# LouChao98/VLGAE

Measured on AMD Instinct MI355X. Metric: sentences/sec, batched inside-outside L=40 B=256, higher is better.
Workload: dtype f32

## Files before the change

vlgae_amd/csrc/vlg_dp_core.h:

```cpp
#pragma once

#if defined(__HIPCC__)
#include <hip/hip_runtime.h>
#define VLG_HD __device__ __forceinline__
#define VLG_HOSTDEV __host__ __device__ inline
#define VLG_HDM __device__ __forceinline__
#define VLG_HOSTDEV_M __host__ __device__
#define VLG_EXP(x) __builtin_amdgcn_exp2f(x)
#define VLG_LOG(x) __builtin_amdgcn_logf(x)
#define VLG_BITS2F(u) __uint_as_float(u)
#define VLG_ATOMIC_ADD(p, v) atomicAdd((p), (v))
#else
#include <cmath>
#include <cstddef>
#include <cstdint>
#include <cstring>
#define VLG_HD static inline
#define VLG_HOSTDEV static inline
#define VLG_HDM inline
#define VLG_HOSTDEV_M
#define VLG_EXP(x) exp2f(x)
#define VLG_LOG(x) log2f(x)
struct float2 { float x, y; };
static inline float2 make_float2(float a, float b) { float2 r; r.x = a; r.y = b; return r; }
static inline float vlg_bits2f(uint32_t u) { float f; std::memcpy(&f, &u, 4); return f; }
#define VLG_BITS2F(u) vlg_bits2f(u)
#define VLG_ATOMIC_ADD(p, v) (*(p) += (v))
#endif

#define VLG_NEGINF (-1e12f)
#define VLG_SR_LOG 0
#define VLG_SR_MAX 1
#define VLG_LOWEST (-3.0e38f)
#if defined(VLG_STAMP) && defined(__HIPCC__) && VLG_STAMP != 2
#define VLG_STAMP_AT(x, k) (x).stamp(k)
#else
#define VLG_STAMP_AT(x, k) ((void)0)
#endif
#if defined(VLG_STAMP) && defined(__HIPCC__)
#define VLG_WSTAMP(x, pass, w, k) (x).wstamp((pass), (w), (k))
#else
#define VLG_WSTAMP(x, pass, w, k) ((void)0)
#endif
#define VLG_LOG2E 1.44269504088896340736f
#define VLG_LN2 0.69314718055994530942f

namespace vlg {

struct F32In {
    using T = float;
    static VLG_HDM float ld(const T* p, size_t i) { return p[i]; }
    static VLG_HDM float2 ld2(const T* p, size_t i) { return make_float2(p[i], p[i + 1]); }
};
#define VLG_POT_FLOOR (-1e30f)
VLG_HD float pot_clamp(float x) { return x > VLG_POT_FLOOR ? x : VLG_POT_FLOOR; }
VLG_HD float2 pot_clamp2(float2 x) { return make_float2(pot_clamp(x.x), pot_clamp(x.y)); }
struct BF16In {
    using T = uint16_t;
    static VLG_HDM float ld(const T* p, size_t i) { return VLG_BITS2F((uint32_t)p[i] << 16); }
    static VLG_HDM float2 ld2(const T* p, size_t i) {
        return make_float2(VLG_BITS2F((uint32_t)p[i] << 16), VLG_BITS2F((uint32_t)p[i + 1] << 16));
    }
};

struct ValSumIn {
    using T = float2;
    static VLG_HDM float ld(const T* p, size_t i) { const float2 v = p[i]; return v.x + v.y; }
};

VLG_HOSTDEV int chart_pitch(int N) { return (N + 1) | 1; }

VLG_HD int dec_idx(int dir, int val, int z) { return (dir * 2 + val) * 2 + z; }

struct DmvCtx {
    int Ne;
    int len;
    int P;
    float2* C;
    float2* I;
    float2* C2;
    float2* I2;
    float* S;
    float* gCc;
    float2* gCi;
    float2* gI;
    float* decs;
    float* gdecs;
    unsigned char* bpS;
    unsigned char* bpC;
    bool walk;
};

template <int SR>
VLG_HD float adj_w(float g, float t, float out, int r, int bp) {
    if (SR == VLG_SR_MAX) return r == bp ? g : 0.f;
    return g * VLG_EXP(fminf(t - out, 0.f));
}

VLG_HD void upd_max(float& m, int& am, float t, int r) {
    if (t > m) { m = t; am = r; }
}

template <int SR>
VLG_HD float fold_term(float m, float s, int am, float t, int rt, bool t_first, int& bp) {
    if (SR == VLG_SR_MAX) {
        const bool take = t_first ? (t >= m) : (t > m);
        bp = take ? rt : am;
        return take ? t : m;
    }
    bp = 0;
    const float d = m - t, e = VLG_EXP(-fabsf(d));
    const float S = d >= 0.f ? s + e : fmaf(s, e, 1.f);
    return fmaxf(m, t) + VLG_LOG(S);
}

#ifndef VLG_DP_LANES_FW
#define VLG_DP_LANES_FW 256
#endif
#ifndef VLG_DP_LANES_BW
#define VLG_DP_LANES_BW 256
#endif
VLG_HD int group_log2(int spans, int w, int nt, int budget) {
    const int cap = budget < nt ? budget : nt;
    int lg = 0;
    while (lg < 6 && (1 << lg) < w && spans * (2 << lg) <= cap) ++lg;
    return lg;
}
#ifndef VLG_MIRROR_RIGHT
#define VLG_MIRROR_RIGHT 1
#endif
#define VLG_GROUP_LOG2_FW(spans, w, nt) group_log2(spans, w, nt, VLG_DP_LANES_FW)
#define VLG_GROUP_LOG2_BW(spans, w, nt) group_log2(spans, w, nt, 512)

struct Sched {
    int first[8];
};
VLG_HD Sched make_sched(int Ne, int lanes, int budget) {
    const int cap = budget < lanes ? budget : lanes;
    Sched s;
    s.first[0] = 1;
    for (int k = 1; k <= 6; ++k) {
        int a = (1 << (k - 1)) + 1, b = Ne - (cap >> k);
        int f = a > b ? a : b;
        if (f < s.first[k - 1]) f = s.first[k - 1];
        s.first[k] = f < Ne ? f : Ne;
    }
    s.first[7] = Ne;
    return s;
}

constexpr int kSpansGeneral = 0, kSpansLong = 1, kSpansShort = 2;
constexpr int kShortN = 41;
constexpr int group_log2_c(int spans, int w, int cap) {
    int lg = 0;
    while (lg < 6 && (1 << lg) < w && spans * (2 << lg) <= cap) ++lg;
    return lg;
}
constexpr bool short_sentence_ok(int n_max, int cap) {
    for (int ne = 2; ne <= n_max; ++ne)
        for (int w = 1; w < ne; ++w) {
            const int lg = group_log2_c(ne - w, w, cap);
            if (((w + (1 << lg) - 1) >> lg) > 3) return false;
        }
    return true;
}
constexpr int short_tmax(int lg_want, int n_max, int cap) {
    int m = 1;
    for (int ne = 2; ne <= n_max; ++ne)
        for (int w = 1; w < ne; ++w) {
            const int lg = group_log2_c(ne - w, w, cap), t = (w + (1 << lg) - 1) >> lg;
            if (lg == lg_want && t > m) m = t;
        }
    return m;
}
static_assert(short_sentence_ok(kShortN, VLG_DP_LANES_FW) && short_sentence_ok(kShortN, VLG_DP_LANES_BW),
// ... 338 lines not shown
                xb[u] = Cf[eB + 2 * rc];
                o_gi[u] = c.gI[eV + rc];
                o_c[u] = c.gCc[eU + rP];
                o_ga[u] = gCif[eA + 2 * rc];
                o_gb[u] = gCif[eB + 2 * rc];
            }
#pragma unroll
            for (int u = 0; u < TU; ++u) {
                const int r = r0 + u * G;
                const bool ok = r < w;
                w0[u] = ok ? adj_w<SR>(gc.x, uu[u] + vv[u].x, oc.x, r, b0) : 0.f;
                w1[u] = ok ? adj_w<SR>(gc.y, uu[u] + vv[u].y, oc.y, r, b1) : 0.f;
            }
            if (!CHUNKED) {
                self[0] = adj_w<SR>(gc.x, su + sv.x, oc.x, selfr, b0);
                self[1] = adj_w<SR>(gc.y, su + sv.y, oc.y, selfr, b1);
            }
            x.lockstep();
            if (!CHUNKED) {
                gi = make_float2(gi_old.x + self[0], gi_old.y + self[1]);
                gs = gi.x + gi.y;
            }
#pragma unroll
            for (int u = 0; u < TU; ++u) {
                const int r = r0 + u * G;
                if (live && r < w) {
                    const float ws = adj_w<SR>(gs, xa[u] + xb[u], Sv, r, bs);
                    if (r != selfr) c.gI[eV + r] = make_float2(o_gi[u].x + w0[u], o_gi[u].y + w1[u]);
                    c.gCc[eU + VLG_MUL24(r, P)] = o_c[u] + (w0[u] + w1[u]);
                    gCif[eA + 2 * r] = o_ga[u] + ws;
                    gCif[eB + 2 * r] = o_gb[u] + ws;
                }
            }
        }
        if (live && rr == 0) c.gI[kO] = gi;
        return;
    }
    for (int r = rr; r < w; r += G) {
        const int rP = VLG_MUL24(r, P);
        const float a = Cf[2 * (eU + rP) + 1];
        const float2 v = c.I[eV + r];
        const float q0 = adj_w<SR>(gc.x, a + v.x, oc.x, r, b0);
        const float q1 = adj_w<SR>(gc.y, a + v.y, oc.y, r, b1);
        if (r != selfr && live) { const float2 t = c.gI[eV + r]; c.gI[eV + r] = make_float2(t.x + q0, t.y + q1); }
        if (live) c.gCc[eU + rP] += q0 + q1;
    }
    self[0] = adj_w<SR>(gc.x, su + sv.x, oc.x, selfr, b0);
    self[1] = adj_w<SR>(gc.y, su + sv.y, oc.y, selfr, b1);
    x.lockstep();
    const float2 gi = make_float2(gi_old.x + self[0], gi_old.y + self[1]);
    const float gs = gi.x + gi.y;
    for (int r = rr; r < w; r += G) {
        const float ws = adj_w<SR>(gs, Cf[eA + 2 * r] + Cf[eB + 2 * r], Sv, r, bs);
        if (live) {
            gCif[eA + 2 * r] += ws;
            gCif[eB + 2 * r] += ws;
        }
    }
    if (live && rr == 0) c.gI[kO] = gi;
}

template <int TM>
struct BwVals {
    float2 oc, sv, vv[TM];
    float Sv, su, uu[TM], xa[TM], xb[TM];
};

template <typename T>
VLG_HD T addr_ld(const char* p, int off = 0) { return *reinterpret_cast<const T*>(p + off); }
template <typename T>
VLG_HD void addr_st(char* p, int off, T v) { *reinterpret_cast<T*>(p + off) = v; }

struct BwAddr {
    const char *vC, *vI, *vS, *vSU, *vUU, *vVV, *vXA, *vXB;
    char *aGc, *aGi, *aI, *aUU, *aVV, *aXA, *aXB;
    int sO8, sO4, sSU, sUU8, sUU4, sVV, sXB;
    int gp8, gp4;
    VLG_HDM void step_vals() { vC += sO8; vI += sO8; vS += sO4; vSU += sSU; vUU += sUU8; vVV += sVV; vXB += sXB; }
    VLG_HDM void step_adj() { aGc += sO4; aGi += sO8; aI += sO8; aUU += sUU4; aVV += sVV; aXB += sXB; }
};

template <int G, typename X>
VLG_HD BwAddr dmv_bw_addr(const DmvCtx& c, int w, int D, int rr, bool right, X& x) {
    const int P = c.P, DW = D + VLG_MUL24(w, P), q = D + rr, qP = D + VLG_MUL24(rr, P);
    const int kO = right ? D + w + 1 : DW, kS = right ? D + w : DW;
    const int iSU = right ? DW + w + 1 : D, iUU = right ? qP + P + w + 1 : qP, iVV = right ? q + 2 : DW + rr;
    const int iXA = q + 1, iXB = DW + rr + 1;
    const int cA = right ? 0 : 4, cB = right ? 4 : 0;
    const char *C = reinterpret_cast<const char*>(c.C), *I = reinterpret_cast<const char*>(c.I), *S = reinterpret_cast<const char*>(c.S);
    char *gCc = reinterpret_cast<char*>(c.gCc), *gCi = reinterpret_cast<char*>(c.gCi), *gI = reinterpret_cast<char*>(c.gI);
    BwAddr a;
    a.vC = x.pin(C + 8 * kO);
    a.vI = x.pin(I + 8 * kO);
    a.vS = x.pin(S + 4 * kS);
    a.vSU = x.pin(C + 8 * iSU + 4);
    a.vUU = x.pin(C + 8 * iUU + 4);
    a.vVV = x.pin(I + 8 * iVV);
    a.vXA = x.pin(C + 8 * iXA + cA);
    a.vXB = x.pin(C + 8 * iXB + cB);
    a.aGc = x.pin(gCc + 4 * kO);
    a.aGi = x.pin(gCi + 8 * kO);
    a.aI = x.pin(gI + 8 * kO);
    a.aUU = x.pin(gCc + 4 * iUU);
    a.aVV = x.pin(gI + 8 * iVV);
    a.aXA = x.pin(gCi + 8 * iXA + cA);
    a.aXB = x.pin(gCi + 8 * iXB + cB);
    a.sO8 = x.uniform(right ? -8 : -8 * P);
    a.sO4 = x.uniform(right ? -4 : -4 * P);
    a.sSU = x.uniform(right ? -8 * (P + 1) : 0);
    a.sUU8 = x.uniform(right ? -8 : 0);
    a.sUU4 = x.uniform(right ? -4 : 0);
    a.sVV = x.uniform(right ? 0 : -8 * P);
    a.sXB = -8 * P;
    a.gp8 = 8 * G * P;
    a.gp4 = 4 * G * P;
    return a;
}

template <int DIR>
struct FwAddr {
    const char *eA, *eB, *eU, *eV, *cX;
    char *oI, *oC, *oS;
    int p8, p4;
    int gp8;
    VLG_HDM void step() {
        eB += p8;
        if (DIR == 0) { eV += p8; oI += p8; oC += p8; oS += p4; }
        else { eU += 8; oI += 8; oC += 8; oS += 4; cX += p8 + 8; }
    }
};

template <int DIR, int G, bool TAPE, typename X>
VLG_HD FwAddr<DIR> dmv_fw_addr(const DmvCtx& c, int w, int D, int rr, X& x) {
    const int P = c.P, DW = D + VLG_MUL24(w, P), q = D + rr, qP = D + VLG_MUL24(rr, P);
    const int kO = DIR == 0 ? DW : D + w + 1;
    const char* C = reinterpret_cast<const char*>(c.C);
    const char* I = reinterpret_cast<const char*>(c.I);
    FwAddr<DIR> a;
    a.eA = x.pin(C + 8 * (q + 1) + (DIR == 0 ? 4 : 0));
    a.eB = x.pin(C + 8 * (DW + rr + 1) + (DIR == 0 ? 0 : 4));
    a.eU = x.pin(C + 8 * (DIR == 0 ? qP : qP + P + w + 1) + 4);
    a.eV = x.pin(I + 8 * (DIR == 0 ? DW + rr : q + 2));
    a.cX = x.pin(C + 8 * (DIR == 0 ? D : DW + w + 1) + 4);
    a.oI = x.pin(reinterpret_cast<char*>(c.I) + 8 * kO);
    a.oC = x.pin(reinterpret_cast<char*>(c.C) + 8 * kO);
    a.oS = nullptr;
    if constexpr (TAPE) a.oS = x.pin(reinterpret_cast<char*>(c.S) + 4 * (DIR == 0 ? DW : D + w));
    a.p8 = x.uniform(8 * P);
    a.p4 = x.uniform(4 * P);
    a.gp8 = 8 * G * P;
    return a;
}

template <int SR, bool BWD, int DIR, int G, int TU, typename X>
VLG_HD void dmv_fw_span_p(const DmvCtx& c, const FwAddr<DIR>& a, int w, bool live, bool root_row, int rr, int D, X& x) {
    const float2 aX = addr_ld<float2>(a.oI);
    const float cX = addr_ld<float>(a.cX);
    float m[3], s[3] = {0.f, 0.f, 0.f};
    int am[3];
    float t[TU][3];
#pragma unroll
    for (int u = 0; u < TU; ++u) {
        const int r = rr + u * G;
        const float av = addr_ld<float>(a.eA, u * G * 8), bv = addr_ld<float>(a.eB, u * G * 8);
        const float uu = addr_ld<float>(a.eU, u * a.gp8);
        const float2 vv = addr_ld<float2>(a.eV, u * G * 8);
        const bool last = u == TU - 1;
        const bool v0 = last ? r < w : true;
        const bool v1 = DIR == 0 ? (v0 && (u == 0 ? r >= 1 : true)) : (last ? r <= w - 2 : true);
        t[u][0] = v0 ? av + bv : VLG_LOWEST;
        t[u][1] = v1 ? uu + vv.x : VLG_LOWEST;
        t[u][2] = v1 ? uu + vv.y : VLG_LOWEST;
    }
#pragma unroll
    for (int k = 0; k < 3; ++k) {
        m[k] = t[0][k];
        am[k] = rr;
        if (SR == VLG_SR_LOG) {
#pragma unroll
            for (int u = 1; u < TU; ++u) m[k] = fmaxf(m[k], t[u][k]);
        } else {
#pragma unroll
            for (int u = 1; u < TU; ++u)
                if (t[u][k] > m[k]) { m[k] = t[u][k]; am[k] = rr + u * G; }
        }
    }
    if (SR == VLG_SR_MAX) x.template allreduce_argmax<3>(m, am, G);
    else x.template allreduce_max<3>(m, G);
    if (SR == VLG_SR_LOG) {
#pragma unroll
        for (int k = 0; k < 3; ++k) {
            s[k] = VLG_EXP(t[0][k] - m[k]);
#pragma unroll
            for (int u = 1; u < TU; ++u) s[k] += VLG_EXP(t[u][k] - m[k]);
        }
        x.template allreduce_sum<3>(s, G);
    }
    const float Sv = SR == VLG_SR_LOG ? m[0] + VLG_LOG(s[0]) : m[0];
    const float2 In = make_float2(aX.x + Sv, aX.y + Sv);
    int b0, b1;
    float Cx = fold_term<SR>(m[1], s[1], am[1], cX + In.x, DIR == 0 ? 0 : w - 1, DIR == 0, b0);
    float Cy = fold_term<SR>(m[2], s[2], am[2], cX + In.y, DIR == 0 ? 0 : w - 1, DIR == 0, b1);
    if (DIR == 1 && root_row && w != c.len) { Cx = VLG_NEGINF; Cy = VLG_NEGINF; }
    if (live && rr == 0) {
        addr_st(a.oI, 0, In);
        addr_st(a.oC, 0, make_float2(Cx, Cy));
        if (BWD) {
            if (SR != VLG_SR_MAX) addr_st(a.oS, 0, Sv);
            if (SR == VLG_SR_MAX) {
                const int DW = D + VLG_MUL24(w, c.P), kO = DIR == 0 ? DW : D + w + 1, kS = DIR == 0 ? DW : D + w;
                c.bpS[kS] = (unsigned char)am[0];
                c.bpC[kO * 2] = (unsigned char)b0;
                c.bpC[kO * 2 + 1] = (unsigned char)b1;
            }
        }
    }
}

template <int SR, bool BWD, int DIR, int LG, int TU, typename X>
VLG_HD void dmv_fw_piece_p(const DmvCtx& c, FwAddr<DIR>& a, int wa, int wb, int slot, int wslot, int rr, int D, X& x) {
    constexpr int G = 1 << LG;
    for (int w = wa; w < wb; ++w) {
        const int spans = x.uniform(c.Ne - w);
        const bool live = slot < spans;
        if (!(X::kSkipDeadWaves && wslot >= spans)) dmv_fw_span_p<SR, BWD, DIR, G, TU>(c, a, w, live, slot == 0, rr, D, x);
        a.step();
        VLG_WSTAMP(x, 0, w, 0);
        x.sync();
        VLG_WSTAMP(x, 0, w, 1);
    }
}

template <int SR, bool BWD, int DIR, int LG, int TM, typename X>
VLG_HD void dmv_fw_dir_p(const DmvCtx& c, int w0, int w1, int t, X& x) {
    constexpr int G = 1 << LG;
    const int rr = t & (G - 1), slot = t >> LG, wslot = (t & ~63) >> LG;
    const int D = slot < c.Ne - w0 ? VLG_MUL24(slot, c.P + 1) : 0;
    FwAddr<DIR> a = dmv_fw_addr<DIR, G, BWD && SR != VLG_SR_MAX>(c, w0, D, rr, x);
#pragma unroll
    for (int k = 1; k <= TM; ++k) {
        const int lo = (k - 1) * G + 1, hi = k == TM ? w1 : k * G + 1;
        const int wa = w0 > lo ? w0 : lo, wb = w1 < hi ? w1 : hi;
        if (k == 1) dmv_fw_piece_p<SR, BWD, DIR, LG, 1>(c, a, wa, wb, slot, wslot, rr, D, x);
        else if (k == 2) dmv_fw_piece_p<SR, BWD, DIR, LG, 2>(c, a, wa, wb, slot, wslot, rr, D, x);
        else dmv_fw_piece_p<SR, BWD, DIR, LG, 3>(c, a, wa, wb, slot, wslot, rr, D, x);
    }
}

template <int SR, bool BWD, int LG, int TM, typename X>
VLG_HD void dmv_fw_segment_p(const DmvCtx& c, int w0, int w1, int tid, int nt, X& x) {
    static_assert(TM >= 1 && TM <= 3, "dmv_fw_dir_p's pieces end at three split points per lane");
    if (w1 <= w0) return;
    const int nd = nt >> 1;
    const bool right = x.uniform(tid >= nd);
    const int t = dir_lane<VLG_MIRROR_RIGHT>(tid, nd, right);
    if (right) dmv_fw_dir_p<SR, BWD, 1, LG, TM>(c, w0, w1, t, x);
    else dmv_fw_dir_p<SR, BWD, 0, LG, TM>(c, w0, w1, t, x);
}

template <int G, int TM, bool XA = true>
VLG_HD void dmv_bw_load_vals(const BwAddr& a, BwVals<TM>& v) {
    v.oc = addr_ld<float2>(a.vC);
    v.Sv = addr_ld<float>(a.vS);
    v.su = addr_ld<float>(a.vSU);
    v.sv = addr_ld<float2>(a.vI);
#pragma unroll
    for (int u = 0; u < TM; ++u) {
        v.uu[u] = addr_ld<float>(a.vUU, u * a.gp8);
        v.vv[u] = addr_ld<float2>(a.vVV, u * G * 8);
        if constexpr (XA) v.xa[u] = addr_ld<float>(a.vXA, u * G * 8);
        v.xb[u] = addr_ld<float>(a.vXB, u * G * 8);
    }
}

template <int TM>
struct BwAdj {
    float ga, o_c[TM], o_gb[TM];
    float2 gb, gi_old, o_gi[TM];
    float e0[TM], e1[TM], es[TM], s0, s1;
};

template <int G, int TM, typename X>
VLG_HD void dmv_bw_span_p1(const BwAddr& a, X& x, const BwVals<TM>& v, BwAdj<TM>& s) {
    s.ga = addr_ld<float>(a.aGc);
    s.gb = addr_ld<float2>(a.aGi);
    s.gi_old = addr_ld<float2>(a.aI);
#pragma unroll
    for (int u = 0; u < TM; ++u) {
        s.o_gi[u] = addr_ld<float2>(a.aVV, u * G * 8);
        s.o_c[u] = addr_ld<float>(a.aUU, u * a.gp4);
        s.o_gb[u] = addr_ld<float>(a.aXB, u * G * 8);
    }
#pragma unroll
    for (int u = 0; u < TM; ++u) {
        s.e0[u] = VLG_EXP(fminf(v.uu[u] + v.vv[u].x - v.oc.x, 0.f));
        s.e1[u] = VLG_EXP(fminf(v.uu[u] + v.vv[u].y - v.oc.y, 0.f));
        s.es[u] = VLG_EXP(fminf(v.xa[u] + v.xb[u] - v.Sv, 0.f));
    }
    s.s0 = VLG_EXP(fminf(v.su + v.sv.x - v.oc.x, 0.f));
    s.s1 = VLG_EXP(fminf(v.su + v.sv.y - v.oc.y, 0.f));
#pragma unroll
    for (int u = 0; u < TM; ++u) {
        x.settle(s.e0[u]);
        x.settle(s.e1[u]);
        x.settle(s.es[u]);
    }
    x.settle(s.s0);
    x.settle(s.s1);
}

template <int G, int TM, typename X>
VLG_HD void dmv_bw_span_p2(const BwAddr& a, int w, bool live, bool gc_ok, int rr, int selfr, X& x, const BwAdj<TM>& s, float (&gxa)[TM]) {
    float2 gc = make_float2(0.f, 0.f);
    if (gc_ok) gc = make_float2(s.gb.x, s.ga + s.gb.y);
    const float self0 = gc.x * s.s0, self1 = gc.y * s.s1;
    x.lockstep();
    const float2 gi = make_float2(s.gi_old.x + self0, s.gi_old.y + self1);
    const float gs = gi.x + gi.y;
#pragma unroll
    for (int u = 0; u < TM; ++u) {
        const int r = rr + u * G;
        if (live && r < w) {
            const float w0 = gc.x * s.e0[u], w1 = gc.y * s.e1[u], ws = gs * s.es[u];
            if (r != selfr) addr_st(a.aVV, u * G * 8, make_float2(s.o_gi[u].x + w0, s.o_gi[u].y + w1));
            addr_st(a.aUU, u * a.gp4, s.o_c[u] + (w0 + w1));
            gxa[u] += ws;
            addr_st(a.aXA, u * G * 8, gxa[u]);
            addr_st(a.aXB, u * G * 8, s.o_gb[u] + ws);
        }
    }
    if (live && rr == 0) addr_st(a.aI, 0, gi);
}

template <int SR, int G, int TM, typename X>
VLG_HD void dmv_bw_segment_p(const DmvCtx& c, int w0, int w1, int tid, int nt, X& x) {
    static_assert(G >= 1 && G <= 64 && TM >= 1 && G * TM <= 64, "a group sits in one wavefront; a lane's last term stays below split point 64");
    if constexpr (SR == VLG_SR_MAX) return;
    if (w1 <= w0) return;
    const int nd = nt >> 1;
    const bool right = x.uniform(tid >= nd);
    const BwLane ln = bw_lane<G>(dir_lane<VLG_MIRROR_RIGHT>(tid, nd, right));
    const int rr = ln.rr, slot = ln.slot, wslot = ln.wslot;
    const int D = slot < c.Ne - w0 ? VLG_MUL24(slot, c.P + 1) : 0;
    const int gc_hi = right && slot == 0 ? 1 : c.Ne;
    BwAddr a = dmv_bw_addr<G>(c, w1 - 1, D, rr, right, x);
    BwVals<TM> v;
    dmv_bw_load_vals<G, TM>(a, v);
    a.step_vals();
    float gxa[TM];
#pragma unroll
    for (int u = 0; u < TM; ++u) gxa[u] = addr_ld<float>(a.aXA, u * G * 8);
    for (int w = w1 - 1; w >= w0; --w) {
        const int spans = x.uniform(c.Ne - w), selfr = x.uniform(right ? w - 1 : 0);
        const bool live = slot < spans;
        const bool body = !(X::kSkipDeadWaves && wslot >= spans);
        BwAdj<TM> s;
        if (body) dmv_bw_span_p1<G, TM>(a, x, v, s);
        dmv_bw_load_vals<G, TM, false>(a, v);
        if (body) dmv_bw_span_p2<G, TM>(a, w, live, live && spans <= gc_hi, rr, selfr, x, s, gxa);
        a.step_vals();
        a.step_adj();
        VLG_WSTAMP(x, 1, w, 0);
        x.sync();
        VLG_WSTAMP(x, 1, w, 1);
    }
}

template <int SR, int DIR, int LG, int LONGSPAN, typename X>
VLG_HD void dmv_bw_width(const DmvCtx& c, int w, int t, int nd, X& x, int dir_rt = 0) {
    constexpr int G = 1 << LG;
    constexpr bool NC = LONGSPAN != 1 && X::kChartsInLds;
    const int per = nd >> LG, rr = t & (G - 1), slot = t >> LG, spans = c.Ne - w;
    const int T = (w + G - 1) >> LG;
    for (int base = 0; base < spans; base += per) {
        const bool live = base + slot < spans;
        const int i = live ? base + slot : 0;
        if (X::kSkipDeadWaves && (base + ((t & ~63) >> LG)) >= spans) continue;
        const int D = VLG_MUL24(i, c.P + 1);
        if constexpr (LONGSPAN == kSpansShort) {
            constexpr int TM = short_tmax(LG, kShortN, VLG_DP_LANES_BW);
            if (TM == 1 || T == 1) dmv_bw_span<SR, DIR, 1, X, false, NC>(c, w, G, D, live, rr, x, 1, dir_rt);
            else if (TM == 2 || T == 2) dmv_bw_span<SR, DIR, 2, X, false, NC>(c, w, G, D, live, rr, x, 1, dir_rt);
            else dmv_bw_span<SR, DIR, 3, X, false, NC>(c, w, G, D, live, rr, x, 1, dir_rt);
        } else if (T == 1) dmv_bw_span<SR, DIR, 1, X, false, NC>(c, w, G, D, live, rr, x, 1, dir_rt);
        else if (T == 2) dmv_bw_span<SR, DIR, 2, X, false, NC>(c, w, G, D, live, rr, x, 1, dir_rt);
        else if (T == 3) dmv_bw_span<SR, DIR, 3, X, false, NC>(c, w, G, D, live, rr, x, 1, dir_rt);
        else if (T == 4) dmv_bw_span<SR, DIR, 4, X, false, NC>(c, w, G, D, live, rr, x, 1, dir_rt);
        else dmv_bw_span<SR, DIR, 4, X, true>(c, w, G, D, live, rr, x, (T + 3) >> 2, dir_rt);
    }
}

struct BwOwn { float2 oc, sv; float Sv, su; };
struct BwChunk { float2 vv[4]; float uu[4], xa[4], xb[4]; };

template <typename T>
VLG_HD T chart_ld(const void* base, int word) {
    return *reinterpret_cast<const T*>(static_cast<const char*>(base) + static_cast<size_t>(static_cast<unsigned>(word) << 2));
}

template <typename X>
VLG_HD void dmv_bw_item_loads(const DmvCtx& c, int w, int G, int D, int r0, int DIR, bool first, BwOwn& own, BwChunk& ch) {
    const int P = c.P, DW = D + VLG_MUL24(w, P);
    const int eA = 2 * (D + 1) + (DIR == 0 ? 1 : 0), eB = 2 * (DW + 1) + (DIR == 0 ? 0 : 1);
    const int eU = DIR == 0 ? D : D + P + w + 1, eV = DIR == 0 ? DW : D + 2;
    if (first) {
        const int kO = DIR == 0 ? DW : D + w + 1, kS = DIR == 0 ? DW : D + w, selfr = DIR == 0 ? 0 : w - 1;
        own.oc = chart_ld<float2>(c.C, 2 * kO);
        own.Sv = chart_ld<float>(c.S, kS);
        own.su = chart_ld<float>(c.C, 2 * (eU + VLG_MUL24(selfr, P)) + 1);
        own.sv = chart_ld<float2>(c.I, 2 * (eV + selfr));
    }
#pragma unroll
    for (int u = 0; u < 4; ++u) {
        const int r = r0 + u * G, rc = r < w ? r : w - 1, rP = VLG_MUL24(rc, P);
        ch.uu[u] = chart_ld<float>(c.C, 2 * (eU + rP) + 1);
        ch.vv[u] = chart_ld<float2>(c.I, 2 * (eV + rc));
        ch.xa[u] = chart_ld<float>(c.C, eA + 2 * rc);
        ch.xb[u] = chart_ld<float>(c.C, eB + 2 * rc);
    }
}

template <int SR, int LG, typename X>
VLG_HD void dmv_bw_segment_s(const DmvCtx& c, int w0, int w1, int tid, int nt, X& x) {
    constexpr int G = 1 << LG;
    if (w1 <= w0) return;
    const int nd = nt >> 1;
    const bool right = x.uniform(tid >= nd);
    const int DIR = right ? 1 : 0;
    const int t = right ? tid - nd : tid;
    const int per = nd >> LG, rr = t & (G - 1), slot = t >> LG, P = c.P;
    float* gCif = reinterpret_cast<float*>(c.gCi);
    auto span_D = [&](int w_, int base_) { return VLG_MUL24(base_ + slot < c.Ne - w_ ? base_ + slot : 0, P + 1); };
    BwOwn own, own_n;
    BwChunk cur, nxt;
    int w = w1 - 1, base = 0, ch = 0;
    dmv_bw_item_loads<X>(c, w, G, span_D(w, 0), rr, DIR, true, own, cur);
    float2 gc = make_float2(0.f, 0.f), gi = make_float2(0.f, 0.f), oc = make_float2(0.f, 0.f);
    float gs = 0.f, Sv = 0.f;
    int b0 = 0, b1 = 0, bs = 0;
    for (;;) {
        const int spans = c.Ne - w, nch = (((w + G - 1) >> LG) + 3) >> 2;
        const bool live = base + slot < spans;
        const int D = span_D(w, base), DW = D + VLG_MUL24(w, P);
        const int eA = 2 * (D + 1) + (DIR == 0 ? 1 : 0), eB = 2 * (DW + 1) + (DIR == 0 ? 0 : 1);
        const int eU = DIR == 0 ? D : D + P + w + 1, eV = DIR == 0 ? DW : D + 2;
        const int kO = DIR == 0 ? DW : D + w + 1, kS = DIR == 0 ? DW : D + w, selfr = DIR == 0 ? 0 : w - 1;
        int wn = w, bn = base, chn = ch + 1;
        bool more = true;
        if (chn == nch) {
            chn = 0;
            bn = base + per;
            if (bn >= spans) { bn = 0; wn = w - 1; more = wn >= w0; }
        }
        const bool width_ends = wn != w;
        const int r0 = rr + ch * (4 * G);
        float ga = 0.f;
        float2 gb = make_float2(0.f, 0.f), gi_old = make_float2(0.f, 0.f);
        if (ch == 0) {
            ga = c.gCc[kO];
            gb = c.gCi[kO];
            gi_old = c.gI[kO];
            if (SR == VLG_SR_MAX) { b0 = c.bpC[kO * 2]; b1 = c.bpC[kO * 2 + 1]; bs = c.bpS[kS]; }
        }
        float o_c[4], o_ga[4], o_gb[4];
        float2 o_gi[4];
#pragma unroll
        for (int u = 0; u < 4; ++u) {
            const int r = r0 + u * G, rc = r < w ? r : w - 1, rP = VLG_MUL24(rc, P);
            o_gi[u] = c.gI[eV + rc];
            o_c[u] = c.gCc[eU + rP];
            o_ga[u] = gCif[eA + 2 * rc];
            o_gb[u] = gCif[eB + 2 * rc];
        }
        if (more) dmv_bw_item_loads<X>(c, wn, G, span_D(wn, bn), rr + chn * (4 * G), DIR, chn == 0, own_n, nxt);
        if (ch == 0) {
            oc = own.oc;
            Sv = own.Sv;
            gc = make_float2(0.f, 0.f);
            if (live && !(DIR == 1 && D == 0 && w != c.len)) gc = make_float2(gb.x, ga + gb.y);
            const float self0 = adj_w<SR>(gc.x, own.su + own.sv.x, oc.x, selfr, b0);
            const float self1 = adj_w<SR>(gc.y, own.su + own.sv.y, oc.y, selfr, b1);
            gi = make_float2(gi_old.x + self0, gi_old.y + self1);
            gs = gi.x + gi.y;
        }
        float q0[4], q1[4];
#pragma unroll
        for (int u = 0; u < 4; ++u) {
            const int r = r0 + u * G;
            const bool ok = r < w;
            q0[u] = ok ? adj_w<SR>(gc.x, cur.uu[u] + cur.vv[u].x, oc.x, r, b0) : 0.f;
            q1[u] = ok ? adj_w<SR>(gc.y, cur.uu[u] + cur.vv[u].y, oc.y, r, b1) : 0.f;
        }
        x.lockstep();
#pragma unroll
        for (int u = 0; u < 4; ++u) {
            const int r = r0 + u * G;
            if (live && r < w) {
                const float ws = adj_w<SR>(gs, cur.xa[u] + cur.xb[u], Sv, r, bs);
                if (r != selfr) c.gI[eV + r] = make_float2(o_gi[u].x + q0[u], o_gi[u].y + q1[u]);
                c.gCc[eU + VLG_MUL24(r, P)] = o_c[u] + (q0[u] + q1[u]);
                gCif[eA + 2 * r] = o_ga[u] + ws;
                gCif[eB + 2 * r] = o_gb[u] + ws;
            }
        }
        if (chn == 0 && live && rr == 0) c.gI[kO] = gi;
        if (width_ends) x.sync();
        if (!more) break;
        if (chn == 0) { own.oc = own_n.oc; own.sv = own_n.sv; own.Sv = own_n.Sv; own.su = own_n.su; }
#pragma unroll
        for (int u = 0; u < 4; ++u) { cur.vv[u] = nxt.vv[u]; cur.uu[u] = nxt.uu[u]; cur.xa[u] = nxt.xa[u]; cur.xb[u] = nxt.xb[u]; }
        w = wn; base = bn; ch = chn;
    }
}

template <int SR, int LG, int LONGSPAN, typename X>
VLG_HD void dmv_bw_segment(const DmvCtx& c, int w0, int w1, int tid, int nt, X& x) {
    const int nd = nt >> 1;
    const bool right = x.uniform(tid >= nd);
// ... 246 lines not shown
    const int T = (w + G - 1) >> LG;
    for (int base = 0; base < spans; base += per) {
        const bool live = base + slot < spans;
        const int i = live ? base + slot : 0;
        if (X::kSkipDeadWaves && (base + ((t & ~63) >> LG)) >= spans) continue;
        const int D = VLG_MUL24(i, c.P + 1);
        if constexpr (SPANS == kSpansShort) {
            constexpr int TM = short_tmax(LG, kShortN, VLG_DP_LANES_BW);
            if (TM == 1 || T == 1) dep_bw_span<SR, DIR, 1>(c, w, G, D, live, rr, x);
            else if (TM == 2 || T == 2) dep_bw_span<SR, DIR, 2>(c, w, G, D, live, rr, x);
            else dep_bw_span<SR, DIR, 3>(c, w, G, D, live, rr, x);
        } else if (T == 1) dep_bw_span<SR, DIR, 1>(c, w, G, D, live, rr, x);
        else if (T == 2) dep_bw_span<SR, DIR, 2>(c, w, G, D, live, rr, x);
        else if (T == 3) dep_bw_span<SR, DIR, 3>(c, w, G, D, live, rr, x);
        else if (T == 4) dep_bw_span<SR, DIR, 4>(c, w, G, D, live, rr, x);
        else dep_bw_span<SR, DIR, 4>(c, w, G, D, live, rr, x, (T + 3) >> 2);
    }
}

template <int SR, int LG, int SPANS, typename X>
VLG_HD void dep_bw_segment(const DepCtx& c, int w0, int w1, int tid, int nt, X& x) {
    const int nd = nt >> 1;
    const bool right = x.uniform(tid >= nd);
    const int t = right ? tid - nd : tid;
    for (int w = w1 - 1; w >= w0; --w) {
        if (right) dep_bw_width<SR, 1, LG, SPANS>(c, w, t, nd, x);
        else dep_bw_width<SR, 0, LG, SPANS>(c, w, t, nd, x);
        x.sync();
    }
}

template <int SR, int SPANS, typename X>
VLG_HD void dep_bw_all(const DepCtx& c, int tid, int nt, X& x) {
    const Sched sc = make_sched(c.Ne, nt >> 1, VLG_DP_LANES_BW);
    dep_bw_segment<SR, 6, SPANS>(c, sc.first[6], sc.first[7], tid, nt, x);
    dep_bw_segment<SR, 5, SPANS>(c, sc.first[5], sc.first[6], tid, nt, x);
    dep_bw_segment<SR, 4, SPANS>(c, sc.first[4], sc.first[5], tid, nt, x);
    dep_bw_segment<SR, 3, SPANS>(c, sc.first[3], sc.first[4], tid, nt, x);
    dep_bw_segment<SR, 2, SPANS>(c, sc.first[2], sc.first[3], tid, nt, x);
    dep_bw_segment<SR, 1, SPANS>(c, sc.first[1], sc.first[2], tid, nt, x);
    dep_bw_segment<SR, 0, SPANS>(c, sc.first[0], sc.first[1], tid, nt, x);
}

template <typename In>
struct MergedIO {
    const typename In::T* dec;
    const typename In::T* attach;
    int N;
    float* gdec;
    float* gatt;
    long long* heads;
    VLG_HDM int out_extent(int) const { return N; }
    VLG_HDM float ld_dec(int i) const { return pot_clamp(In::ld(dec, i)); }
    VLG_HDM float2 ld_attach(int h, int ch) const { return pot_clamp2(In::ld2(attach, ((size_t)h * N + ch) * 2)); }
    VLG_HDM void st_attach(int h, int ch, float2 g) const {
        if (gatt) *reinterpret_cast<float2*>(gatt + ((size_t)h * N + ch) * 2) = g;
        if (heads && g.x + g.y != 0.f) heads[ch] = h;
    }
    VLG_HDM bool wants_dec() const { return gdec != nullptr; }
    VLG_HDM void st_dec(int h, int k, float g) const { gdec[h * 8 + k] = g; }
    VLG_HDM void clear_heads(int tid, int nt) const {
        if (heads) for (int i = tid; i < N; i += nt) heads[i] = 0;
    }
};

template <typename In>
struct RuleIO {
    const typename In::T* rule;
    const typename In::T* dec;
    const typename In::T* root;
    const long long* token;
    const unsigned char* head_mask;
    int L, T;
    float fill;
    float* g_rule;
    float* g_dec;
    float* g_root;
    long long* heads;
    VLG_HDM int out_extent(int Ne) const { return Ne; }
    VLG_HDM float ld_dec(int i) const {
        const int h = i >> 3, k = i & 7;
        if (h == 0) return (k >> 2) == 1 ? 0.f : VLG_NEGINF;
        return pot_clamp(In::ld(dec, (h - 1) * 8 + k));
    }
    VLG_HDM size_t rule_index(int h, int ch) const {
        return ((((size_t)(h - 1) * T + (size_t)token[ch - 1]) * 2 + (ch < h ? 0 : 1)) * 2);
    }
    VLG_HDM float2 ld_attach(int h, int ch) const {
        if (ch == 0) return make_float2(VLG_NEGINF, VLG_NEGINF);
        if (h == 0) return make_float2(VLG_NEGINF, pot_clamp(In::ld(root, (size_t)token[ch - 1])));
        if (head_mask && head_mask[h - 1]) return make_float2(fill, fill);
        return pot_clamp2(In::ld2(rule, rule_index(h, ch)));
    }
    VLG_HDM void st_attach(int h, int ch, float2 g) const {
        if (heads && g.x + g.y != 0.f) heads[ch] = h;
        if (!g_rule || ch == 0 || h == ch) return;
        if (h == 0) { if (g.y != 0.f) VLG_ATOMIC_ADD(g_root + token[ch - 1], g.y); return; }
        if (head_mask && head_mask[h - 1]) return;
        float* p = g_rule + rule_index(h, ch);
        if (g.x != 0.f) VLG_ATOMIC_ADD(p, g.x);
        if (g.y != 0.f) VLG_ATOMIC_ADD(p + 1, g.y);
    }
    VLG_HDM bool wants_dec() const { return g_dec != nullptr; }
    VLG_HDM void st_dec(int h, int k, float g) const {
        if (h >= 1) g_dec[(h - 1) * 8 + k] = g;
    }
    VLG_HDM void clear_heads(int tid, int nt) const {
        if (heads) for (int i = tid; i < L + 1; i += nt) heads[i] = 0;
    }
};

VLG_HD int walk_entry(int kind, int a, int b, int v) { return kind | (a << 2) | (b << 10) | (v << 18); }

VLG_HD void dmv_walk(const DmvCtx& c, float g) {
    const int P = c.P;
    int* stack = reinterpret_cast<int*>(c.gCc);
    int top = 0;
    int e = walk_entry(1, 0, c.len, 1);
    for (;;) {
        const int kind = e & 3, a = (e >> 2) & 255, b = (e >> 10) & 255, v = (e >> 18) & 1;
        if (kind < 2 && a == b) {
            c.gdecs[a * 4 + kind * 2 + v] = g;
            if (top == 0) break;
            e = stack[--top];
            continue;
        }
        int sib;
        if (kind == 0) {
            const int r = c.bpC[(a * P + b) * 2 + v];
            sib = walk_entry(0, b + r, b, 1);
            e = walk_entry(2, a, b + r, v);
        } else if (kind == 1) {
            const int r = c.bpC[(a * P + b + 1) * 2 + v];
            sib = walk_entry(1, a + 1 + r, b, 1);
            e = walk_entry(3, a, a + 1 + r, v);
        } else if (kind == 2) {
            reinterpret_cast<float*>(c.gI + a * P + b)[v] = g;
            const int r = c.bpS[a * P + b];
            sib = walk_entry(1, b, b + r, 1);
            e = walk_entry(0, a, b + r + 1, 0);
        } else {
            reinterpret_cast<float*>(c.gI + a * P + b + 1)[v] = g;
            const int r = c.bpS[a * P + b];
            sib = walk_entry(1, a, a + r, 0);
            e = walk_entry(0, b, a + r + 1, 1);
        }
        stack[top++] = sib;
    }
}

template <int SR, bool BWD, int LONGSPAN = false, typename IO, typename X>
VLG_HD void dmv_run(const DmvCtx& c, const IO& io, float glogZ, float* logZ, int tid, int nt, X& x) {
    const int Ne = c.Ne, P = c.P, len = c.len;
    const float2 zz = make_float2(VLG_NEGINF, VLG_NEGINF), oo = make_float2(0.f, 0.f);
    const int NN = Ne * Ne;
    const float inv_ne = 1.0f / (float)Ne;
    constexpr int KC = 4;
    for (int base = 0; base < NN; base += KC * nt) {
        float2 areg[KC];
#pragma unroll
        for (int k = 0; k < KC; ++k) {
            const int idx = base + tid + k * nt;
            const int h = (int)(((float)idx + 0.5f) * inv_ne), ch = idx - h * Ne;
            areg[k] = (idx < NN && ch != h) ? io.ld_attach(h, ch) : zz;
        }
        if (base == 0) {
            for (int i = tid; i < Ne * 8; i += nt) c.decs[i] = io.ld_dec(i) * VLG_LOG2E;
            for (int i = tid; i < Ne * P; i += nt) {
                c.C[i] = zz;
                c.I[i] = zz;
            }
            x.sync();
        }
#pragma unroll
        for (int k = 0; k < KC; ++k) {
            const int idx = base + tid + k * nt;
            if (idx >= NN) continue;
            const int h = (int)(((float)idx + 0.5f) * inv_ne), ch = idx - h * Ne;
            const float* d = c.decs + h * 8;
            if (ch == h) {
                c.C[h * P + h] = make_float2(d[1], d[3]);
                c.C[h * P + h + 1] = make_float2(d[5], d[7]);
            } else if (ch < h) {
                c.I[h * P + ch] = make_float2(fmaf(areg[k].x, VLG_LOG2E, d[0]), fmaf(areg[k].y, VLG_LOG2E, d[2]));
            } else {
                c.I[h * P + ch + 1] = make_float2(fmaf(areg[k].x, VLG_LOG2E, d[4]), fmaf(areg[k].y, VLG_LOG2E, d[6]));
            }
        }
    }
    x.sync();
#if defined(VLG_STAMP) && defined(__HIPCC__)
    unsigned long long st_body = 0, st_sync = 0, st_t0 = __builtin_amdgcn_s_memtime(), st_stage = 0, st_end = 0;
    unsigned long long st_bbody = 0, st_bsync = 0;
    {
        const unsigned long long a = __builtin_amdgcn_s_memtime();
        dmv_fw_all<SR, BWD, LONGSPAN>(c, tid, nt, x);
        st_body += __builtin_amdgcn_s_memtime() - a;
    }
#else
    dmv_fw_all<SR, BWD, LONGSPAN>(c, tid, nt, x);
#endif
    if (tid == 0) *logZ = c.C[len + 1].y * VLG_LN2;
    if (!BWD) return;
    if (c.C2 != c.C) {
        for (int i = tid; i < Ne * P; i += nt) {
            c.C2[i] = c.C[i];
            c.I2[i] = c.I[i];
        }
        x.sync();
    }
    for (int i = tid; i < Ne * P; i += nt) {
        c.gI[i] = oo;
        if (SR != VLG_SR_MAX) { c.gCc[i] = 0.f; c.gCi[i] = oo; }
    }
    if (SR == VLG_SR_MAX) for (int i = tid; i < Ne * 4; i += nt) c.gdecs[i] = 0.f;
    x.sync();
    DmvCtx cb = c;
    cb.C = c.C2;
    cb.I = c.I2;
    if (SR == VLG_SR_MAX) {
        if (tid == 0) dmv_walk(cb, glogZ);
        x.sync();
    } else {
    if (tid == 0) c.gCc[len + 1] = glogZ;
    x.sync();
#if defined(VLG_STAMP) && defined(__HIPCC__)
    {
        const unsigned long long a = __builtin_amdgcn_s_memtime();
        dmv_bw_all<SR, LONGSPAN>(cb, tid, nt, x);
        st_bbody += __builtin_amdgcn_s_memtime() - a;
    }
    st_end = __builtin_amdgcn_s_memtime();
#else
    dmv_bw_all<SR, LONGSPAN>(cb, tid, nt, x);
#endif
    }
    io.clear_heads(tid, nt);
    x.sync();
    const int E = io.out_extent(Ne);
    const float inv_e = 1.0f / (float)E;
    for (int idx = tid; idx < E * E; idx += nt) {
        const int h = (int)(((float)idx + 0.5f) * inv_e), ch = idx - h * E;
        float2 g = oo;
        if (h < Ne && ch < Ne) {
            if (ch < h) g = c.gI[h * P + ch];
            else if (ch > h) g = c.gI[h * P + ch + 1];
        }
        io.st_attach(h, ch, g);
    }
    if (io.wants_dec()) {
        for (int idx = tid; idx < E * 4; idx += nt) {
            const int h = idx >> 2, dir = (idx >> 1) & 1, v = idx & 1;
            float g = 0.f;
            if (h < Ne) {
                const int q = h * P + h + dir;
                g = SR == VLG_SR_MAX ? c.gdecs[h * 4 + dir * 2 + v] : (v == 1 ? c.gCc[q] : 0.f) + reinterpret_cast<const float*>(c.gCi + q)[v];
            }
            io.st_dec(h, (dir * 2 + v) * 2 + 1, g);
        }
        constexpr int GL = 4;
        for (int base = 0; base < E * 2; base += nt / GL) {
            const int grp = base + tid / GL, rr = tid % GL;
            const int h = grp >> 1, dir = grp & 1;
            float sum[2] = {0.f, 0.f};
            if (grp < E * 2 && h < Ne) {
                const float2* row = c.gI + h * P + (dir == 0 ? 0 : h + 2);
                const int n = dir == 0 ? h : Ne - 1 - h;
                for (int k = rr; k < n; k += GL) { sum[0] += row[k].x; sum[1] += row[k].y; }
            }
            x.template allreduce_sum<2>(sum, GL);
            if (grp < E * 2 && rr == 0) {
                io.st_dec(h, (dir * 2 + 0) * 2, sum[0]);
                io.st_dec(h, (dir * 2 + 1) * 2, sum[1]);
            }
        }
    }
#if defined(VLG_STAMP) && defined(__HIPCC__)
    x.sync();
    if ((tid & 63) == 0) {
        float* o = io.gdec + (size_t)(io.N - 1 - (tid >> 6)) * 8;
        o[0] = (float)st_body; o[1] = (float)st_sync; o[2] = (float)st_bbody; o[3] = (float)st_bsync;
        o[4] = (float)(st_end - st_t0); o[5] = (float)st_stage; o[6] = 0.f; o[7] = 0.f;
        float* o2 = io.gdec + (size_t)(io.N - 1 - 8 - (tid >> 6)) * 8;
        for (int k = 0; k < 8; ++k) o2[k] = (float)x.acc[k];
    }
#endif
}

VLG_HD void dep_walk(const DepCtx& c, float g) {
    const int P = c.P;
    int* stack = reinterpret_cast<int*>(c.gCc);
    int top = 0;
    int e = walk_entry(1, 0, c.len, 0);
    for (;;) {
        const int kind = e & 3, a = (e >> 2) & 255, b = (e >> 10) & 255;
        if (kind < 2 && a == b) {
            if (top == 0) break;
            e = stack[--top];
            continue;
        }
        int sib;
        if (kind == 0) {
            const int r = c.bpC[a * P + b];
            sib = walk_entry(0, b + r, b, 0);
            e = walk_entry(2, a, b + r, 0);
        } else if (kind == 1) {
            const int r = c.bpC[a * P + b + 1];
            sib = walk_entry(1, a + 1 + r, b, 0);
            e = walk_entry(3, a, a + 1 + r, 0);
        } else if (kind == 2) {
            c.gI[a * P + b] = g;
            const int r = c.bpS[b * P + a];
            sib = walk_entry(1, b, b + r, 0);
            e = walk_entry(0, a, b + r + 1, 0);
        } else {
            c.gI[a * P + b + 1] = g;
            const int r = c.bpS[a * P + b];
            sib = walk_entry(1, a, a + r, 0);
            e = walk_entry(0, b, a + r + 1, 0);
        }
        stack[top++] = sib;
    }
}

template <int SR, bool BWD, typename In, int SPANS = kSpansGeneral, typename X>
VLG_HD void dep_run(const DepCtx& c, const typename In::T* arc, int N, float glogZ, float* logZ, float* garc,
                    long long* heads, int tid, int nt, X& x) {
    const int Ne = c.Ne, P = c.P, len = c.len;
    for (int i = tid; i < Ne * P; i += nt) {
        c.C[i] = VLG_NEGINF;
        c.I[i] = VLG_NEGINF;
        if (BWD) {
            c.gI[i] = 0.f;
            if (SR != VLG_SR_MAX) { c.gCc[i] = 0.f; c.gCi[i] = 0.f; }
        }
    }
    x.sync();
    for (int idx = tid; idx < Ne * Ne; idx += nt) {
        const int h = idx / Ne, ch = idx - h * Ne;
        if (ch == h) {
            c.C[h * P + h] = 0.f;
            c.C[h * P + h + 1] = 0.f;
        } else {
            const float a = pot_clamp(In::ld(arc, (size_t)h * N + ch)) * VLG_LOG2E;
            if (ch < h) c.I[h * P + ch] = a;
            else c.I[h * P + ch + 1] = a;
        }
    }
    x.sync();
    dep_fw_all<SR, BWD, SPANS>(c, tid, nt, x);
    if (tid == 0) *logZ = c.C[len + 1] * VLG_LN2;
    if (!BWD) return;
    if (SR == VLG_SR_MAX) {
        if (tid == 0) dep_walk(c, glogZ);
        x.sync();
    } else {
        if (tid == 0) c.gCc[len + 1] = glogZ;
        x.sync();
        dep_bw_all<SR, SPANS>(c, tid, nt, x);
    }
    if (heads) {
        for (int i = tid; i < N; i += nt) heads[i] = 0;
        x.sync();
    }
    for (int idx = tid; idx < N * N; idx += nt) {
        const int h = idx / N, ch = idx - h * N;
        float g = 0.f;
        if (h < Ne && ch < Ne && ch != h) {
            g = ch < h ? c.gI[h * P + ch] : c.gI[h * P + ch + 1];
            if (SR != VLG_SR_MAX) {
                const int i = ch < h ? ch : h, w = ch < h ? h - ch : ch - h;
                g += dep_self<SR>(c, i * (P + 1), w, ch < h ? 0 : 1);
            }
        }
        if (garc) garc[idx] = g;
        if (heads && g != 0.f) heads[ch] = h;
    }
}

VLG_HOSTDEV size_t align16(size_t x) { return (x + 15) & ~(size_t)15; }

struct Region {
    size_t off;
    bool lds;
};

struct Carver {
    size_t lds = 0, ws = 0;
    VLG_HOSTDEV_M Region take(size_t bytes, bool in_lds) {
        Region r;
        r.lds = in_lds;
        if (in_lds) { r.off = lds; lds = align16(lds + bytes); }
        else { r.off = ws; ws = align16(ws + bytes); }
        return r;
    }
};

struct DmvLayout {
    Region C, I, S, bpS, bpC, gCc, gCi, gI, decs, gdecs;
    Region C_in, I_in;
    size_t lds_bytes, ws_bytes;
    VLG_HOSTDEV_M DmvLayout(int N, bool bwd, bool is_max, int mode, bool walk = false) {
        const size_t cells = (size_t)N * chart_pitch(N);
        Carver k;
        if (walk) {
            const bool v = mode < 2, a2 = mode < 1;
            C = k.take(cells * 8, v);
            I = k.take(cells * 8, v);
            S = k.take(0, v);
            bpS = k.take(cells, v);
            bpC = k.take(cells * 2, v);
            gCc = k.take((2 * (size_t)N + 4) * 4, true);
            gCi = k.take(0, true);
            gI = k.take(cells * 8, a2);
            decs = k.take((size_t)N * 32, true);
            gdecs = k.take((size_t)N * 16, true);
            C_in = C;
            I_in = I;
        } else {
            const bool v = mode < 1, a1 = mode < 3, a2 = mode < 2;
            const bool overlay = bwd && mode == 1;
            if (overlay) {
                gCc = k.take(cells * 4, true);
                gCi = k.take(cells * 8, true);
                gI = k.take(cells * 8, true);
                C_in.lds = true; C_in.off = 0;
                I_in.lds = true; I_in.off = align16(cells * 8);
            }
            C = k.take(cells * 8, v);
            I = k.take(cells * 8, v);
            S = k.take(bwd ? cells * 4 : 0, v);
            bpS = k.take(bwd && is_max ? cells : 0, v);
            bpC = k.take(bwd && is_max ? cells * 2 : 0, v);
            if (!overlay) {
                gCc = k.take(bwd ? cells * 4 : 0, a1);
// ... 92 lines not shown
```

Before: 4.764 million.

## Hold loop-invariant span terms in registers across widths in forward and backward DP

In the forward span loop, terms other than the last that stay the same across successive widths are now loaded once per piece into registers instead of reloaded every width. The backward loop is split per direction, and the running gradient accumulators for the invariant side (xa plus uu or vv) are kept in registers, which drops their per-width reloads. The backward loop also uses fma and adds settle calls. Stamp instrumentation gains extra timing fields. The risks are higher register pressure and a correctness dependence on those addresses really being invariant across widths.

```diff
diff --git a/vlgae_amd/csrc/vlg_dp_core.h b/vlgae_amd/csrc/vlg_dp_core.h
--- a/vlgae_amd/csrc/vlg_dp_core.h
+++ b/vlgae_amd/csrc/vlg_dp_core.h
@@ -8,6 +8,7 @@
 #define VLG_HOSTDEV_M __host__ __device__
 #define VLG_EXP(x) __builtin_amdgcn_exp2f(x)
 #define VLG_LOG(x) __builtin_amdgcn_logf(x)
+#define VLG_MULADD(a, b, c) __builtin_fmaf((a), (b), (c))
 #define VLG_BITS2F(u) __uint_as_float(u)
 #define VLG_ATOMIC_ADD(p, v) atomicAdd((p), (v))
 #else
@@ -21,6 +22,7 @@
 #define VLG_HOSTDEV_M
 #define VLG_EXP(x) exp2f(x)
 #define VLG_LOG(x) log2f(x)
+#define VLG_MULADD(a, b, c) ((a) * (b) + (c))
 struct float2 { float x, y; };
 static inline float2 make_float2(float a, float b) { float2 r; r.x = a; r.y = b; return r; }
 static inline float vlg_bits2f(uint32_t u) { float f; std::memcpy(&f, &u, 4); return f; }
@@ -665,8 +667,26 @@
     return a;
 }
 
-template <int SR, bool BWD, int DIR, int G, int TU, typename X>
-VLG_HD void dmv_fw_span_p(const DmvCtx& c, const FwAddr<DIR>& a, int w, bool live, bool root_row, int rr, int D, X& x) {
+template <int DIR, int NH>
+struct FwHeld {
+    float av[NH > 0 ? NH : 1];
+    float uu[NH > 0 ? NH : 1];
+    float2 vv[NH > 0 ? NH : 1];
+};
+
+template <int DIR, int G, int NH>
+VLG_HD void dmv_fw_load_held(const FwAddr<DIR>& a, FwHeld<DIR, NH>& h) {
+#pragma unroll
+    for (int u = 0; u < NH; ++u) {
+        h.av[u] = addr_ld<float>(a.eA, u * G * 8);
+        if constexpr (DIR == 0) h.uu[u] = addr_ld<float>(a.eU, u * a.gp8);
+        else h.vv[u] = addr_ld<float2>(a.eV, u * G * 8);
+    }
+}
+
+template <int SR, bool BWD, int DIR, int G, int TU, int NH, typename X>
+VLG_HD void dmv_fw_span_p(const DmvCtx& c, const FwAddr<DIR>& a, const FwHeld<DIR, NH>& h, int w, bool live, bool root_row, int rr, int D, X& x) {
+    static_assert(NH == 0 || NH == TU - 1, "every term but the last is held, or none");
     const float2 aX = addr_ld<float2>(a.oI);
     const float cX = addr_ld<float>(a.cX);
     float m[3], s[3] = {0.f, 0.f, 0.f};
@@ -675,9 +695,10 @@
 #pragma unroll
     for (int u = 0; u < TU; ++u) {
         const int r = rr + u * G;
-        const float av = addr_ld<float>(a.eA, u * G * 8), bv = addr_ld<float>(a.eB, u * G * 8);
-        const float uu = addr_ld<float>(a.eU, u * a.gp8);
-        const float2 vv = addr_ld<float2>(a.eV, u * G * 8);
+        const bool held = u < NH;
+        const float av = held ? h.av[u] : addr_ld<float>(a.eA, u * G * 8), bv = addr_ld<float>(a.eB, u * G * 8);
+        const float uu = held && DIR == 0 ? h.uu[u] : addr_ld<float>(a.eU, u * a.gp8);
+        const float2 vv = held && DIR == 1 ? h.vv[u] : addr_ld<float2>(a.eV, u * G * 8);
         const bool last = u == TU - 1;
         const bool v0 = last ? r < w : true;
         const bool v1 = DIR == 0 ? (v0 && (u == 0 ? r >= 1 : true)) : (last ? r <= w - 2 : true);
@@ -733,10 +754,14 @@
 template <int SR, bool BWD, int DIR, int LG, int TU, typename X>
 VLG_HD void dmv_fw_piece_p(const DmvCtx& c, FwAddr<DIR>& a, int wa, int wb, int slot, int wslot, int rr, int D, X& x) {
     constexpr int G = 1 << LG;
+    constexpr int NH = G > 1 ? TU - 1 : 0;
+    if (NH > 0 && wa >= wb) return;
+    FwHeld<DIR, NH> h;
+    dmv_fw_load_held<DIR, G, NH>(a, h);
     for (int w = wa; w < wb; ++w) {
         const int spans = x.uniform(c.Ne - w);
         const bool live = slot < spans;
-        if (!(X::kSkipDeadWaves && wslot >= spans)) dmv_fw_span_p<SR, BWD, DIR, G, TU>(c, a, w, live, slot == 0, rr, D, x);
+        if (!(X::kSkipDeadWaves && wslot >= spans)) dmv_fw_span_p<SR, BWD, DIR, G, TU, NH>(c, a, h, w, live, slot == 0, rr, D, x);
         a.step();
         VLG_WSTAMP(x, 0, w, 0);
         x.sync();
@@ -771,7 +796,7 @@
     else dmv_fw_dir_p<SR, BWD, 0, LG, TM>(c, w0, w1, t, x);
 }
 
-template <int G, int TM, bool XA = true>
+template <int DIR, int G, int TM, bool FIRST>
 VLG_HD void dmv_bw_load_vals(const BwAddr& a, BwVals<TM>& v) {
     v.oc = addr_ld<float2>(a.vC);
     v.Sv = addr_ld<float>(a.vS);
@@ -779,10 +804,27 @@
     v.sv = addr_ld<float2>(a.vI);
 #pragma unroll
     for (int u = 0; u < TM; ++u) {
-        v.uu[u] = addr_ld<float>(a.vUU, u * a.gp8);
-        v.vv[u] = addr_ld<float2>(a.vVV, u * G * 8);
-        if constexpr (XA) v.xa[u] = addr_ld<float>(a.vXA, u * G * 8);
+        if constexpr (FIRST || DIR != 0) v.uu[u] = addr_ld<float>(a.vUU, u * a.gp8);
+        if constexpr (FIRST || DIR != 1) v.vv[u] = addr_ld<float2>(a.vVV, u * G * 8);
+        if constexpr (FIRST) v.xa[u] = addr_ld<float>(a.vXA, u * G * 8);
         v.xb[u] = addr_ld<float>(a.vXB, u * G * 8);
+    }
+}
+
+template <int DIR, int TM>
+struct BwHeld {
+    float gxa[TM];
+    float guu[TM];
+    float2 gvv[TM];
+};
+
+template <int DIR, int G, int TM>
+VLG_HD void dmv_bw_load_held(const BwAddr& a, BwHeld<DIR, TM>& h) {
+#pragma unroll
+    for (int u = 0; u < TM; ++u) {
+        h.gxa[u] = addr_ld<float>(a.aXA, u * G * 8);
+        if constexpr (DIR == 0) h.guu[u] = addr_ld<float>(a.aUU, u * a.gp4);
+        else h.gvv[u] = addr_ld<float2>(a.aVV, u * G * 8);
     }
 }
 
@@ -793,15 +835,15 @@
     float e0[TM], e1[TM], es[TM], s0, s1;
 };
 
-template <int G, int TM, typename X>
+template <int DIR, int G, int TM, typename X>
 VLG_HD void dmv_bw_span_p1(const BwAddr& a, X& x, const BwVals<TM>& v, BwAdj<TM>& s) {
     s.ga = addr_ld<float>(a.aGc);
     s.gb = addr_ld<float2>(a.aGi);
     s.gi_old = addr_ld<float2>(a.aI);
 #pragma unroll
     for (int u = 0; u < TM; ++u) {
-        s.o_gi[u] = addr_ld<float2>(a.aVV, u * G * 8);
-        s.o_c[u] = addr_ld<float>(a.aUU, u * a.gp4);
+        if constexpr (DIR == 0) s.o_gi[u] = addr_ld<float2>(a.aVV, u * G * 8);
+        else s.o_c[u] = addr_ld<float>(a.aUU, u * a.gp4);
         s.o_gb[u] = addr_ld<float>(a.aXB, u * G * 8);
     }
 #pragma unroll
@@ -822,8 +864,9 @@
     x.settle(s.s1);
 }
 
-template <int G, int TM, typename X>
-VLG_HD void dmv_bw_span_p2(const BwAddr& a, int w, bool live, bool gc_ok, int rr, int selfr, X& x, const BwAdj<TM>& s, float (&gxa)[TM]) {
+template <int DIR, int G, int TM, typename X>
+VLG_HD void dmv_bw_span_p2(const BwAddr& a, int w, bool live, bool gc_ok, int rr, X& x, const BwAdj<TM>& s, BwHeld<DIR, TM>& h) {
+    const int selfr = DIR == 0 ? 0 : w - 1;
     float2 gc = make_float2(0.f, 0.f);
     if (gc_ok) gc = make_float2(s.gb.x, s.ga + s.gb.y);
     const float self0 = gc.x * s.s0, self1 = gc.y * s.s1;
@@ -834,15 +877,54 @@
     for (int u = 0; u < TM; ++u) {
         const int r = rr + u * G;
         if (live && r < w) {
-            const float w0 = gc.x * s.e0[u], w1 = gc.y * s.e1[u], ws = gs * s.es[u];
-            if (r != selfr) addr_st(a.aVV, u * G * 8, make_float2(s.o_gi[u].x + w0, s.o_gi[u].y + w1));
-            addr_st(a.aUU, u * a.gp4, s.o_c[u] + (w0 + w1));
-            gxa[u] += ws;
-            addr_st(a.aXA, u * G * 8, gxa[u]);
-            addr_st(a.aXB, u * G * 8, s.o_gb[u] + ws);
+            float w0 = gc.x * s.e0[u], w1 = gc.y * s.e1[u];
+            x.settle(w0);
+            x.settle(w1);
+            if constexpr (DIR == 0) {
+                if (r != selfr) addr_st(a.aVV, u * G * 8, make_float2(s.o_gi[u].x + w0, s.o_gi[u].y + w1));
+                h.guu[u] += (w0 + w1);
+                addr_st(a.aUU, u * a.gp4, h.guu[u]);
+            } else {
+                if (r != selfr) {
+                    h.gvv[u] = make_float2(h.gvv[u].x + w0, h.gvv[u].y + w1);
+                    addr_st(a.aVV, u * G * 8, h.gvv[u]);
+                }
+                addr_st(a.aUU, u * a.gp4, s.o_c[u] + (w0 + w1));
+            }
+            h.gxa[u] = VLG_MULADD(gs, s.es[u], h.gxa[u]);
+            addr_st(a.aXA, u * G * 8, h.gxa[u]);
+            addr_st(a.aXB, u * G * 8, VLG_MULADD(gs, s.es[u], s.o_gb[u]));
         }
     }
     if (live && rr == 0) addr_st(a.aI, 0, gi);
+}
+
+template <int SR, int DIR, int G, int TM, typename X>
+VLG_HD void dmv_bw_dir_p(const DmvCtx& c, int w0, int w1, int t, X& x) {
+    const BwLane ln = bw_lane<G>(t);
+    const int rr = ln.rr, slot = ln.slot, wslot = ln.wslot;
+    const int D = slot < c.Ne - w0 ? VLG_MUL24(slot, c.P + 1) : 0;
+    const int gc_hi = DIR == 1 && slot == 0 ? 1 : c.Ne;
+    BwAddr a = dmv_bw_addr<G>(c, w1 - 1, D, rr, DIR == 1, x);
+    BwVals<TM> v;
+    dmv_bw_load_vals<DIR, G, TM, true>(a, v);
+    a.step_vals();
+    BwHeld<DIR, TM> h;
+    dmv_bw_load_held<DIR, G, TM>(a, h);
+    for (int w = w1 - 1; w >= w0; --w) {
+        const int spans = x.uniform(c.Ne - w);
+        const bool live = slot < spans;
+        const bool body = !(X::kSkipDeadWaves && wslot >= spans);
+        BwAdj<TM> s;
+        if (body) dmv_bw_span_p1<DIR, G, TM>(a, x, v, s);
+        dmv_bw_load_vals<DIR, G, TM, false>(a, v);
+        if (body) dmv_bw_span_p2<DIR, G, TM>(a, w, live, live && spans <= gc_hi, rr, x, s, h);
+        a.step_vals();
+        a.step_adj();
+        VLG_WSTAMP(x, 1, w, 0);
+        x.sync();
+        VLG_WSTAMP(x, 1, w, 1);
+    }
 }
 
 template <int SR, int G, int TM, typename X>
@@ -852,31 +934,9 @@
     if (w1 <= w0) return;
     const int nd = nt >> 1;
     const bool right = x.uniform(tid >= nd);
-    const BwLane ln = bw_lane<G>(dir_lane<VLG_MIRROR_RIGHT>(tid, nd, right));
-    const int rr = ln.rr, slot = ln.slot, wslot = ln.wslot;
-    const int D = slot < c.Ne - w0 ? VLG_MUL24(slot, c.P + 1) : 0;
-    const int gc_hi = right && slot == 0 ? 1 : c.Ne;
-    BwAddr a = dmv_bw_addr<G>(c, w1 - 1, D, rr, right, x);
-    BwVals<TM> v;
-    dmv_bw_load_vals<G, TM>(a, v);
-    a.step_vals();
-    float gxa[TM];
-#pragma unroll
-    for (int u = 0; u < TM; ++u) gxa[u] = addr_ld<float>(a.aXA, u * G * 8);
-    for (int w = w1 - 1; w >= w0; --w) {
-        const int spans = x.uniform(c.Ne - w), selfr = x.uniform(right ? w - 1 : 0);
-        const bool live = slot < spans;
-        const bool body = !(X::kSkipDeadWaves && wslot >= spans);
-        BwAdj<TM> s;
-        if (body) dmv_bw_span_p1<G, TM>(a, x, v, s);
-        dmv_bw_load_vals<G, TM, false>(a, v);
-        if (body) dmv_bw_span_p2<G, TM>(a, w, live, live && spans <= gc_hi, rr, selfr, x, s, gxa);
-        a.step_vals();
-        a.step_adj();
-        VLG_WSTAMP(x, 1, w, 0);
-        x.sync();
-        VLG_WSTAMP(x, 1, w, 1);
-    }
+    const int t = dir_lane<VLG_MIRROR_RIGHT>(tid, nd, right);
+    if (right) dmv_bw_dir_p<SR, 1, G, TM>(c, w0, w1, t, x);
+    else dmv_bw_dir_p<SR, 0, G, TM>(c, w0, w1, t, x);
 }
 
 template <int SR, int DIR, int LG, int LONGSPAN, typename X>
@@ -1429,6 +1489,9 @@
 template <int SR, bool BWD, int LONGSPAN = false, typename IO, typename X>
 VLG_HD void dmv_run(const DmvCtx& c, const IO& io, float glogZ, float* logZ, int tid, int nt, X& x) {
     const int Ne = c.Ne, P = c.P, len = c.len;
+#if defined(VLG_STAMP) && defined(__HIPCC__)
+    const unsigned long long st_in = __builtin_amdgcn_s_memtime();
+#endif
     const float2 zz = make_float2(VLG_NEGINF, VLG_NEGINF), oo = make_float2(0.f, 0.f);
     const int NN = Ne * Ne;
     const float inv_ne = 1.0f / (float)Ne;
@@ -1467,12 +1530,13 @@
     }
     x.sync();
 #if defined(VLG_STAMP) && defined(__HIPCC__)
-    unsigned long long st_body = 0, st_sync = 0, st_t0 = __builtin_amdgcn_s_memtime(), st_stage = 0, st_end = 0;
-    unsigned long long st_bbody = 0, st_bsync = 0;
+    unsigned long long st_body = 0, st_sync = 0, st_t0 = __builtin_amdgcn_s_memtime(), st_stage = st_t0 - st_in, st_end = 0;
+    unsigned long long st_bbody = 0, st_bsync = 0, st_mid0 = 0, st_mid = 0;
     {
         const unsigned long long a = __builtin_amdgcn_s_memtime();
         dmv_fw_all<SR, BWD, LONGSPAN>(c, tid, nt, x);
-        st_body += __builtin_amdgcn_s_memtime() - a;
+        st_mid0 = __builtin_amdgcn_s_memtime();
+        st_body += st_mid0 - a;
     }
 #else
     dmv_fw_all<SR, BWD, LONGSPAN>(c, tid, nt, x);
@@ -1504,6 +1568,7 @@
 #if defined(VLG_STAMP) && defined(__HIPCC__)
     {
         const unsigned long long a = __builtin_amdgcn_s_memtime();
+        st_mid = a - st_mid0;
         dmv_bw_all<SR, LONGSPAN>(cb, tid, nt, x);
         st_bbody += __builtin_amdgcn_s_memtime() - a;
     }
@@ -1553,11 +1618,12 @@
         }
     }
 #if defined(VLG_STAMP) && defined(__HIPCC__)
+    const unsigned long long st_out = SR == VLG_SR_MAX ? 0 : __builtin_amdgcn_s_memtime() - st_end;
     x.sync();
     if ((tid & 63) == 0) {
         float* o = io.gdec + (size_t)(io.N - 1 - (tid >> 6)) * 8;
         o[0] = (float)st_body; o[1] = (float)st_sync; o[2] = (float)st_bbody; o[3] = (float)st_bsync;
-        o[4] = (float)(st_end - st_t0); o[5] = (float)st_stage; o[6] = 0.f; o[7] = 0.f;
+        o[4] = (float)(st_end - st_t0); o[5] = (float)st_stage; o[6] = (float)st_mid; o[7] = (float)st_out;
         float* o2 = io.gdec + (size_t)(io.N - 1 - 8 - (tid >> 6)) * 8;
         for (int k = 0; k < 8; ++k) o2[k] = (float)x.acc[k];
     }
```

Measured after the change: 5.163 million, median of 6. 8.4% higher.
